# zgspose/PAVENet

Hardware: AMD Instinct MI355X
Metric: clips/sec (T=7, 800x1344) fwd (higher is better)
Workload: dtype f32 (exact 3-term bf16 split on the bf16 MFMA)

## Files before the change

### include/pave_hip.h

```cpp
#ifndef PAVE_HIP_H_
#define PAVE_HIP_H_

#include <stdint.h>

#ifdef __cplusplus
extern "C" {
#endif

#define PAVE_OK 0
#define PAVE_E_ARG (-1)
#define PAVE_E_LAUNCH (-2)
#define PAVE_E_STEP (-3)
#define PAVE_E_UNSUPPORTED (-4)

#define PAVE_ABI_VERSION 21
int pave_abi_version(void);
const char* pave_last_error(void);

int pave_ms_deform_attn_forward_f32(const float* value, const int64_t* spatial_shapes,
                                    const int64_t* level_start, const float* sampling_loc,
                                    const float* attn_weight, float* out, int bs, int S, int M,
                                    int D, int L, int Lq, int P, int im2col_step, void* stream);
int pave_ms_deform_attn_forward_f64(const double* value, const int64_t* spatial_shapes,
                                    const int64_t* level_start, const double* sampling_loc,
// ... 246 lines not shown
int pave_gemm_fp16_act_f32(const void* a, int a_is_f16, const void* w_plane, const float* bias,
                           const float* residual, const float* gamma, const float* beta, float eps, void* out,
                           int out_is_f16, long long M, int K, int N, int relu, void* stream);

int pave_gemm_bf16x3_ex_f32(const float* a, const float* a_bias, const void* w_planes,
                            const float* bias, const float* residual, long long residual_rows,
                            float* out, float* out2, int n_split, long long M, int K, int N,
                            int relu, int nplanes, void* stream);

int pave_ref_update_f32(const float* tmp, const float* ref, float* out, long long n, float eps,
                        void* stream);

int pave_groupnorm_nhwc_f32(const float* x, const float* gamma, const float* beta, float* y,
                            long long y_batch_stride, int N, int HW, int C, int G, float eps,
                            double* partial, int nchunks, float* ab, void* stream);

typedef struct pave_gn_level {
  const float* x;
  const float* gamma;
  const float* beta;
  float* y;
  long long y_batch_stride;
  int HW;
  int nchunks;
  float eps;
} pave_gn_level;
int pave_groupnorm_levels_nhwc_f32(const pave_gn_level* levels, int nlev, int N, int C, int G, double* partial,
                                   float* ab, void* stream);

int pave_gemm_bf16x3_cat_f32(const float* a, long long K1, const float* a2, const void* w_planes,
                             const float* bias, const float* residual, float* out, long long M, int K,
                             int N, int relu, int nplanes, void* stream);

int pave_gemm_bf16x3_grouped_f32(const float* a, long long lda, const void* w_planes, const float* bias,
                                 float* out, long long M, int K, int N, int group_n, int relu,
                                 int nplanes, void* stream);

int pave_gemm_bf16x3_ln_f32(const float* a, const void* w_planes, const float* bias,
                            const float* residual, const float* gamma, const float* beta, float eps,
                            float* out, long long M, int K, int N, int nplanes, void* stream);

int pave_conv3x3_split_f32(const float* x, const void* w_planes, const float* bias,
                           const float* residual, float* y, int N, int H, int W, int Cin, int Cout,
                           int stride, int relu, int nplanes, void* stream);

long long pave_conv3x3_splitk_workspace_bytes(int N, int H, int W, int Cin, int Cout, int stride);
int pave_conv3x3_splitk_f32(const float* x, const void* w_planes, const float* bias,
                            const float* residual, float* y, int N, int H, int W, int Cin, int Cout,
                            int stride, int relu, void* workspace, long long workspace_bytes,
                            int nplanes, void* stream);

long long pave_gemm_splitk_workspace_bytes(long long M, int K, int N);
int pave_gemm_bf16x3_splitk_f32(const float* a, const void* w_planes, const float* bias, const float* residual,
                                float* out, long long M, int K, int N, int relu, int nplanes, void* workspace,
                                long long workspace_bytes, void* stream);

int pave_set_form_policy(int policy);
int pave_get_form_policy(void);

#define PAVE_FORM_ROWS 0
#define PAVE_FORM_ROWS_SPLITK 1
#define PAVE_FORM_ROWS_TILE 2
#define PAVE_FORM_LN 3
#define PAVE_FORM_CONV3X3 4
#define PAVE_FORM_CONV1X1S 5
#define PAVE_FORM_ENCPROJ 6
// ... 56 lines not shown
```

### pavenet_amd/backbones.py

```python
import torch
import torch.nn as nn
import torch.nn.functional as F

from .bricks import BaseModule, build_norm_layer
from .registry import MMDET_MODELS


class BasicBlock(nn.Module):
    expansion = 1

    def __init__(self, inplanes, planes, stride=1, dilation=1, downsample=None, style='pytorch',
                 norm_cfg=dict(type='BN')):
        super().__init__()
        self.conv1 = nn.Conv2d(inplanes, planes, 3, stride, dilation, dilation, bias=False)
        self.bn1 = build_norm_layer(norm_cfg, planes)[1]
        self.conv2 = nn.Conv2d(planes, planes, 3, 1, 1, bias=False)
        self.bn2 = build_norm_layer(norm_cfg, planes)[1]
        self.relu = nn.ReLU(inplace=True)
        self.downsample = downsample
        self.pairs = (('conv1', 'bn1', True), ('conv2', 'bn2', False))


class Bottleneck(nn.Module):
    expansion = 4
# ... 50 lines not shown
        self.norm_eval = norm_eval
        self.style = style
        block, stage_blocks = self.arch_settings[depth]
        stage_blocks = stage_blocks[:num_stages]
        self.conv1 = nn.Conv2d(in_channels, stem_channels, 7, 2, 3, bias=False)
        self.bn1 = build_norm_layer(norm_cfg, stem_channels)[1]
        self.relu = nn.ReLU(inplace=True)
        self.maxpool = nn.MaxPool2d(kernel_size=3, stride=2, padding=1)
        self.res_layers = []
        inplanes = stem_channels
        for i, nb in enumerate(stage_blocks):
            planes = base_channels * 2**i
            layers = []
            for b in range(nb):
                stride = strides[i] if b == 0 else 1
                downsample = None
                if b == 0 and (stride != 1 or inplanes != planes * block.expansion):
                    downsample = nn.Sequential(
                        nn.Conv2d(inplanes, planes * block.expansion, 1, stride, bias=False),
                        build_norm_layer(norm_cfg, planes * block.expansion)[1])
                layers.append(block(inplanes, planes, stride, dilations[i], downsample, style,
                                    norm_cfg))
                inplanes = planes * block.expansion
            name = f'layer{i + 1}'
            self.add_module(name, nn.Sequential(*layers))
            self.res_layers.append(name)
        self.feat_dim = inplanes
        self._folded = None
        self.channels_last = True
        self.fused_tail_max_k = 256
        self.fused_ds_max_k = 128
        self.chain_stage64 = True
        self.chain_mode = 'full'
        self.deterministic_conv3x3 = False

    def init_weights(self):
        for m in self.modules():
            if isinstance(m, nn.Conv2d):
                nn.init.kaiming_normal_(m.weight, mode='fan_out', nonlinearity='relu')
            elif isinstance(m, (nn.BatchNorm2d, nn.GroupNorm)):
                nn.init.constant_(m.weight, 1)
                nn.init.constant_(m.bias, 0)
        for m in self.modules():
            if isinstance(m, Bottleneck):
                nn.init.constant_(m.bn3.weight, 0)
            elif isinstance(m, BasicBlock):
                nn.init.constant_(m.bn2.weight, 0)
        self._is_init = True

    def _params_key(self):
        from .bricks import SourceKey, module_tensors
        return SourceKey(module_tensors(self))

    def _stem_folded(self):
        from .bricks import SourceKey
        bn = self.bn1
        key = SourceKey([self.conv1.weight, bn.weight, bn.bias, bn.running_mean, bn.running_var])
        hit = self.__dict__.get('_stem_cache')
        if hit is None or hit[0] != key:
            mf = torch.channels_last if self.channels_last else torch.contiguous_format
            with torch.no_grad():
                hit = (key, tuple(t.contiguous(memory_format=mf) if t.dim() == 4 else t
                                  for t in _fold(self.conv1, self.bn1)))
            self.__dict__['_stem_cache'] = hit
        return hit[1]

# ... 17 lines not shown
                                and w.shape[1] % 32 == 0:
                            f[(name, bi, 'conv3_kn')] = w.flatten(1).t().contiguous()
                    if blk.downsample is not None:
                        w, b = _fold(blk.downsample[0], blk.downsample[1])
                        f[(name, bi, 'ds')] = (w.contiguous(memory_format=mf), b)
                        w3_kn = f.get((name, bi, 'conv3_kn'))
                        if w3_kn is not None and w.shape[1] % 32 == 0 and \
                                w3_kn.shape[0] + w.shape[1] <= self.fused_ds_max_k:
                            f[(name, bi, 'tail_ds_kn')] = (
                                torch.cat([w3_kn, w.flatten(1).t()], 0).contiguous(),
                                f[(name, bi, 'conv3')][1] + b)
        self._folded = (key, f)
        return f

    @staticmethod
    def _stem_split(x_nchw, w):
        from . import ops
        from .bricks import _split_cached, fused_mode, get_gemm_mode
        if not fused_mode() or torch.is_grad_enabled() or not x_nchw.is_cuda \
                or x_nchw.dtype != torch.float32 or tuple(w.shape) != (64, 3, 7, 7) \
                or x_nchw.shape[1] != 3 or x_nchw.shape[3] < 8 or not x_nchw.is_contiguous():
            return None
        wp = _split_cached(w, 'stem7x7', lambda planes: ops.split_stem7x7_weight(w.detach(), planes))
        if x_nchw.shape[3] % 4 or x_nchw.data_ptr() % 16:
            return ops.conv7x7s2_nchw_split(ops.repitch_rows(x_nchw), wp, valid_w=x_nchw.shape[3])
        return ops.conv7x7s2_nchw_split(x_nchw, wp)

    @staticmethod
    def _ds_bias(f, name, bi):
        key = (name, bi, 'ds_b3')
        if key not in f:
            f[key] = f[(name, bi, 'ds')][1] + f[(name, bi, 'conv3')][1]
        return f[key]

    @staticmethod
    def _as_rows(x):
        n, c, h, w = x.shape
        return x.permute(0, 2, 3, 1).reshape(-1, c), (n, h, w)

    @staticmethod
    def _as_map(rows, nhw):
        n, h, w = nhw
        return rows.view(n, h, w, rows.shape[-1]).permute(0, 3, 1, 2)

    def _stage64_chain_ok(self, name, x, f):
        from .bricks import _GEMM, fused_mode
        blocks = list(getattr(self, name))
        if blocks[0].downsample is not None and (name, 0, 'tail_ds_kn') not in f:
            return False
        if not (self.chain_stage64 and fused_mode() and not torch.is_grad_enabled()
                and x.is_contiguous(memory_format=torch.channels_last)
                and x.shape[0] * x.shape[2] * x.shape[3] >= _GEMM['min_rows']
                and all(isinstance(b, Bottleneck) for b in blocks)):
            return False
        for bi, blk in enumerate(blocks):
            c1, c2, c3 = blk.conv1, blk.conv2, blk.conv3
            if not (c1.out_channels == 64 and c1.stride == (1, 1)
                    and tuple(c2.weight.shape) == (64, 64, 3, 3) and c2.stride == (1, 1)
                    and c2.dilation == (1, 1) and c2.padding == (1, 1) and c2.groups == 1
                    and tuple(c3.weight.shape[:2]) == (256, 64)):
                return False
            if blk.downsample is not None and not (
                    bi == 0 and blk.downsample[0].stride == (1, 1)
                    and blk.downsample[0].in_channels == 64):
                return False
            if blk.downsample is None and c1.in_channels != 256:
# ... 54 lines not shown
        if c2.dilation[0] == 1 and c2.padding[0] == 1 and c2.stride[0] == c2.stride[1] \
                and not torch.is_grad_enabled():
            wsplit = split_conv_weight(w2)
        from .bricks import fused_mode, small_split_ok
        split3 = blk.downsample is None and (
            split_gemm_ok(rows, w3.flatten(1))
            or (wsplit is not None and fused_mode() and small_split_ok(rows, w3.flatten(1))))
        if split3:
            w3_kn = None
        if wsplit is not None:
            from .bricks import get_gemm_mode
            y = ops.conv3x3_split(y, wsplit, b2, stride=c2.stride[0], relu=True,
                                  fp16=get_gemm_mode() == 'fp16')
            b2 = None
        elif taps is not None and c2.dilation[0] == 1 and c2.padding[0] == 1:
            y = ops.conv3x3_nhwc(y, taps, b2, stride=c2.stride[0], relu=True)
            b2 = None
        else:
            y = F.conv2d(y, w2, None, c2.stride, c2.padding, c2.dilation)
            if w3_kn is None and not split3:
                ops.bias_act_rows_(y, b2, None, relu=True)
                b2 = None
        yrows, onhw = self._as_rows(y)
        if blk.downsample is not None:
            wd, bd = f[(name, bi, 'ds')]
            s = blk.downsample[0].stride[0]
            tail = f.get((name, bi, 'tail_ds_kn'))
            from .bricks import _GEMM, _split_weight, fused_mode, small_split_ok
            w3_split = b2 is None and (split_gemm_ok(yrows, w3.flatten(1)) or small_split_ok(yrows, w3.flatten(1)))
            if (s > 1 and tail is None and fused_mode() and not torch.is_grad_enabled()
                    and wd.shape[0] % 128 == 0 and wd.shape[1] % 64 == 0
                    and (yrows.shape[0] >= _GEMM['min_rows'] or w3_split)
                    and (w3_kn is not None or w3_split or split_gemm_ok(yrows, w3.flatten(1)))):
                idt = ops.conv1x1_strided_split(x, _split_weight(wd.flatten(1)),
                                                self._ds_bias(f, name, bi), stride=s)
                idt, _ = self._as_rows(idt)
                if w3_split or split_gemm_ok(yrows, w3.flatten(1)):
                    out = linear_rows(yrows, w3.flatten(1), None, relu=True, residual=idt,
                                      inplace_residual=True, a_bias=b2)
                else:
                    out = ops.rows_gemm_bias_res_act(yrows, w3_kn, None, idt, relu=True, out=idt,
                                                     a_bias=b2)
                return self._as_map(out, onhw)
            xs = x if s == 1 else x[:, :, ::s, ::s].contiguous(memory_format=torch.channels_last)
            xrows, _ = self._as_rows(xs)
            from .bricks import _split_cached
            if tail is not None and b2 is None and fused_mode() \
                    and not torch.is_grad_enabled() \
                    and tail[0].shape[0] % 32 == 0 and tail[0].shape[1] % 64 == 0 \
                    and yrows.shape[1] % 16 == 0:
                wcat = _split_cached(tail[0], 'tail_cat', lambda planes: ops.split_weight_bf16x3(
                    tail[0].t().contiguous(), planes))
                out = ops.gemm_bf16x3_cat(yrows, xrows, wcat, tail[1], None, relu=True)
            elif tail is not None:
                out = ops.rows_gemm_bias_res_act(yrows, tail[0], tail[1], None, relu=True,
                                                 a_bias=b2, a2=xrows)
            elif split_gemm_ok(xrows, wd.flatten(1)) and \
                    (w3_kn is not None or split_gemm_ok(yrows, w3.flatten(1))):
                idt = linear_rows(xrows, wd.flatten(1), self._ds_bias(f, name, bi))
                if split_gemm_ok(yrows, w3.flatten(1)):
                    out = linear_rows(yrows, w3.flatten(1), None, relu=True, residual=idt,
                                      inplace_residual=True, a_bias=b2)
                else:
                    out = ops.rows_gemm_bias_res_act(yrows, w3_kn, None, idt, relu=True, out=idt,
                                                     a_bias=b2)
            else:
# ... 412 lines not shown
```

### pavenet_amd/csrc/pave_gemm_dma.hip

```cpp
#include <hip/hip_runtime.h>
#include <type_traits>
#include <stdint.h>

#include "pave_hip.h"
#include "pave_internal.h"
#include "pave_enc_math.h"

namespace {

typedef __bf16 bf16x8 __attribute__((ext_vector_type(8)));
typedef float f32x16 __attribute__((ext_vector_type(16)));
typedef unsigned u32x4 __attribute__((ext_vector_type(4)));
typedef float f32x4 __attribute__((ext_vector_type(4)));

constexpr int QBM = 128;
constexpr int QNS = 3;
constexpr int QCST = 36;

struct QConv {
  int H, W, Cin, Ho, Wo, stride;
  unsigned rcp;
};
struct QOut {
  float* out2;
// ... 145 lines not shown
__device__ __forceinline__ void gemm_q_body(
    const float* __restrict__ A, const uint16_t* __restrict__ Wp, const float* __restrict__ bias,
    const float* residual, float* out, const int M, const int K, const int N, const int relu,
    const float* __restrict__ a_bias, const QConv g, const QOut os, const QLn ln,
    const float* __restrict__ A2 = nullptr, const int tile_m0 = -1, const int tile_n0 = 0,
    const QEpi* epi = nullptr) {
  constexpr int NWAVE = 4 * WN;
  constexpr int BN = WN * TN * 32;
  constexpr int BM = QBM * RM;
  constexpr bool AH = (IO & 1) != 0, OH = (IO & 2) != 0;
  static_assert(!AH || (PL == 1 && KIND == 0 && !ABIAS && RM == 1), "fp16 A rows: fp16 operand mode, plain rows");
  static_assert(!OH || (PL == 1 && !LNORM && EPI == 0 && !HT && RM == 1), "fp16 output: plain epilogue");
  constexpr int A_STAGE = AH ? BM * 32 : BM * 64;
  static_assert(RM == 1 || (RM == 2 && WN == 1 && !WIDE && !LNORM && EPI == 0), "two row tiles per wave: narrow form");
  static_assert(PL == 3 || PL == 1, "operand planes: 3 (bf16 split) or 1 (fp16)");
  constexpr int W_STAGE = PL * BN * 32;
  constexpr int STAGE = A_STAGE + W_STAGE;
  constexpr int NA = A_STAGE / 1024;
  constexpr int NWI = W_STAGE / 1024;
  constexpr int NDI = NA + NWI;
  constexpr int QMAX = (NDI + NWAVE - 1) / NWAVE;
  constexpr int QMIN = NDI / NWAVE;
  constexpr int QA = (NA + NWAVE - 1) / NWAVE;
  constexpr int NS = WIDE ? 2 : QNS;
  constexpr int EPI_OFF = 0;
  constexpr int STAT_OFF = NS * STAGE;
  constexpr int TQ = WIDE ? 2 : (HT ? 1 : TN);
  static_assert(!HT || (TN == 2 && WN == 1 && RM == 1 && !WIDE && !LNORM && EPI == 0 && PL == 3),
                "half-tail form: 64-column planes, one row tile per wave, 3 planes");
  static_assert(!WIDE || (TN == 8 && WN == 1 && !ABIAS), "wide form: 32 x 256 per wave");
  constexpr int ABOFF = STAT_OFF + (LNORM ? 2 * QBM * WN * 4 : 0);
  static_assert(NA % NWAVE == 0, "A DMA instructions divide evenly over the waves");
  static_assert(!LNORM || KIND == 0, "LayerNorm epilogue: plain row GEMM only");
  static_assert(KIND >= 0 && KIND <= 4, "row source");
  extern __shared__ __attribute__((aligned(1024))) unsigned char smem[];

  const int tid = threadIdx.x, lane = tid & 63;
  const int wave = __builtin_amdgcn_readfirstlane(tid >> 6);
  const int wm = wave / WN, wn = wave % WN;
  const int lr = lane & 31, kh = lane >> 5;
  const int ntiles = N / BN;
  const int ttot = ((M + BM - 1) / BM) * ntiles;
  const int per = ttot >> 3, rem = ttot & 7;
  const unsigned lds0 = (unsigned)(size_t)(__attribute__((address_space(3))) unsigned char*)smem;
  const int s0 = os.ks_slabs > 0 ? (int)blockIdx.y * os.ks_slabs : 0;
  const int nslabs = os.ks_slabs > 0 ? min(os.ks_slabs, K / 16 - s0) : K / 16;
  const long long w_slab = (long long)PL * N * 32;
  const unsigned char* const w_base = reinterpret_cast<const unsigned char*>(Wp);

  int m0 = 0, n0 = 0;
  unsigned a_voff[QA];
  unsigned a2_voff[QA];
  const unsigned char* a2_base = reinterpret_cast<const unsigned char*>(A2);
  int a_iy0[QA], a_ix0[QA];
  const float* a_img[QA];
  unsigned a_mask[QA];
  i32x4 a_rsrc;
  if (KIND == 1) {
    const unsigned long long ab = reinterpret_cast<unsigned long long>(A);
    a_rsrc.x = __builtin_amdgcn_readfirstlane((int)(unsigned)ab);
    a_rsrc.y = __builtin_amdgcn_readfirstlane((int)(unsigned)(ab >> 32) & 0xffff);
    a_rsrc.z = __builtin_amdgcn_readfirstlane(
        (int)((unsigned)(M / (g.Ho * g.Wo)) * (unsigned)g.H * (unsigned)g.W * (unsigned)g.Cin * 4u));
    a_rsrc.w = 0x00020000;
  }
  unsigned w_voff[QMAX - QA];
  const unsigned char* a_base = reinterpret_cast<const unsigned char*>(A);

  auto setup_tile = [&](const int t) {
    const int xcd = t & 7, idx = t >> 3;
    const int lb = xcd * per + (xcd < rem ? xcd : rem) + idx;
    m0 = (lb / ntiles) * BM;
    n0 = (lb % ntiles) * BN;
    if (tile_m0 >= 0) m0 = tile_m0, n0 = tile_n0;
#pragma unroll
    for (int q = 0; q < QA; ++q) {
      const int d = wave + NWAVE * q;
      const int r = AH ? d * 32 + (lane >> 1) : d * 16 + (lane >> 2);
      const int c = AH ? (lane & 1) ^ ((r >> 3) & 1) : (lane & 3) ^ ((r >> 2) & 3);
      long long gm = (long long)m0 + r;
      if (gm >= M) gm = M - 1;
      if (KIND == 0 && AH) {
        a_voff[q] = (unsigned)(((gm - m0) * (g.H > 0 ? g.H : K) + c * 8) * 2);
      } else if (KIND == 0) {
        a_voff[q] = (unsigned)(((gm - m0) * (g.H > 0 ? g.H : K) + c * 4) * 4);
      } else if (KIND == 4) {
        a_voff[q] = (unsigned)(((gm - m0) * g.Cin + c * 4) * 4);
        a2_voff[q] = (unsigned)(((gm - m0) * (K - g.Cin) + c * 4) * 4);
      } else {
        const unsigned ur = (unsigned)gm, gy = ur / (unsigned)g.Wo;
        const int ox = (int)(ur - gy * (unsigned)g.Wo);
        const int n = (int)(gy / (unsigned)g.Ho);
        const int oy = (int)(gy - (unsigned)n * (unsigned)g.Ho);
        if (KIND == 3) {
          a_voff[q] = (unsigned)(((((long long)n * g.H + oy * g.stride) * g.W + ox * g.stride) * K + c * 4) * 4);
        } else if (KIND == 1) {
          const int iy0 = oy * g.stride - 1, ix0 = ox * g.stride - 1;
          a_voff[q] = (unsigned)(((((long long)n * g.H + iy0) * g.W + ix0) * g.Cin + c * 4) * 4);
          unsigned mk = 0;
#pragma unroll
          for (int t = 0; t < 9; ++t) {
            const int iy = iy0 + t / 3, ix = ix0 + t % 3;
            mk |= (iy >= 0 && iy < g.H && ix >= 0 && ix < g.W) ? (1u << t) : 0u;
          }
          a_mask[q] = mk;
        } else {
          a_iy0[q] = oy * g.stride - 1;
          a_ix0[q] = ox * g.stride - 1;
          a_img[q] = A + (long long)n * g.H * g.W * g.Cin + c * 4;
        }
      }
    }
    if (KIND == 0 && AH)
      a_base = reinterpret_cast<const unsigned char*>(A) +
               ((long long)m0 * (g.H > 0 ? g.H : K) + (g.W > 0 ? (long long)(n0 / g.W) * K : 0)) * 2;
    else if (KIND == 0)
      a_base = reinterpret_cast<const unsigned char*>(A + (long long)(PAVE_PROBE_CACHED_A() ? 0 : m0) * (g.H > 0 ? g.H : K) +
                                                      (g.W > 0 ? (long long)(n0 / g.W) * K : 0));
    if (KIND == 4) {
      a_base = reinterpret_cast<const unsigned char*>(A + (long long)m0 * g.Cin);
      a2_base = reinterpret_cast<const unsigned char*>(A2 + (long long)m0 * (K - g.Cin));
    }
#pragma unroll
    for (int q = QA; q < QMAX; ++q) {
      const int j = wave + NWAVE * (q - QA);
      const int p = j / (NWI / PL), row = (j % (NWI / PL)) * 32 + (lane >> 1);
      const int h = (lane & 1) ^ ((row >> 3) & 1);
      w_voff[q - QA] = (unsigned)((((long long)p * N + n0 + row) * 32 + h * 16));
    }
  };
  auto issue = [&](const int rel, const int stage) {
    const int slab = rel + s0;
    const unsigned sl = lds0 + stage * STAGE;
#pragma unroll
    for (int q = 0; q < QA; ++q) {
      const unsigned dst = sl + (wave + NWAVE * q) * 1024;
      if (KIND == 1) {
        const int tap = g.rcp ? (int)__umulhi((unsigned)slab, g.rcp) : slab;
        const int c0 = (slab - tap * (g.Cin >> 4)) * 16;
        const int ky = (tap * 11) >> 5, kx = tap - ky * 3;
        const unsigned toff = (unsigned)(((ky * g.W + kx) * g.Cin + c0) * 4);
        const bool ok = (a_mask[q] >> tap) & 1u;
        dma16_buf(ok ? a_voff[q] + toff : 0xffffff00u, a_rsrc, dst);
      } else if (KIND == 2) {
        const int k0 = slab * 16;
        const int tap = k0 / g.Cin, c0 = k0 - tap * g.Cin;
        const int ky = tap / 3, kx = tap - ky * 3;
        const int iy = a_iy0[q] + ky, ix = a_ix0[q] + kx;
        const bool ok = tap < 9 && iy >= 0 && iy < g.H && ix >= 0 && ix < g.W;
        const float* src = ok ? a_img[q] + ((long long)iy * g.W + ix) * g.Cin + c0
                              : reinterpret_cast<const float*>(g_zero_chunk);
        dma16_flat(src, dst);
      } else if (KIND == 4) {
        const int s1 = g.Cin >> 4;
        if (slab < s1) dma16(a_voff[q], a_base + (long long)slab * 64, dst);
        else dma16(a2_voff[q], a2_base + (long long)(slab - s1) * 64, dst);
      } else {
        dma16(a_voff[q], a_base + (long long)slab * (AH ? 32 : 64), dst);
      }
    }
#pragma unroll
    for (int q = QA; q < QMAX; ++q) {
      const int j = wave + NWAVE * (q - QA);
      if (NWI % NWAVE == 0 || j < NWI)
        dma16(w_voff[q - QA], w_base + slab * w_slab, sl + A_STAGE + j * 1024);
    }
  };

  const int sw = (lr >> 2) & 3;
  const int a_rd0 = AH ? (wm * 32 + lr) * 32 + ((kh ^ ((lr >> 3) & 1)) * 16)
                       : (wm * 32 * RM + lr) * 64 + (((2 * kh) ^ sw) * 16);
  const int a_rd1 = a_rd0 ^ 16;
  const int w_rd = A_STAGE + (wn * TN * 32 + lr) * 32 + ((kh ^ ((lr >> 3) & 1)) * 16);

  f32x16 acc[RM * TN];
  f32x4 raw[RM][2];
  u32x4 apl[2][RM][PL];
  u32x4 wf[2][PL][TQ];
  const float* const ab_lds = reinterpret_cast<const float*>(smem + ABOFF);

  auto read_raw = [&](const int stage) {
    const unsigned char* st = smem + stage * STAGE;
#pragma unroll
    for (int rt = 0; rt < RM; ++rt) {
      raw[rt][0] = *reinterpret_cast<const f32x4*>(st + a_rd0 + rt * 2048);
      if constexpr (!AH) raw[rt][1] = *reinterpret_cast<const f32x4*>(st + a_rd1 + rt * 2048);
// ... 1310 lines not shown
      break;
    case PAVE_FORM_LN: {
      bool lnpass, sk, wide;
      ln_form(M, Kp, Np, policy, dv, &lnpass, &sk, &wide);
      if (lnpass) *order = sk ? PAVE_ORDER_KSPLIT_LNPASS : PAVE_ORDER_TILE_LNPASS;
      else *order = wide ? PAVE_ORDER_TILE : PAVE_ORDER_TILE_LN8;
      break;
    }
    case PAVE_FORM_CONV3X3:
      if (dv != PAVE_DV_FIRST_GEN) splitk_plan(M, Kp, Np, policy, &parts, &per);
      if (parts > 1) *order = PAVE_ORDER_SPLITK, *ksplit = parts;
      break;
    default:
      break;
  }
  return PAVE_OK;
}
int pave_internal_splitk_reduce(const float* ws, int parts, long long M, int n, const float* bias,
                                const float* residual, int relu, float* out, void* stream) {
  const long long total4 = M * n / 4;
  return pave_launch<splitk_reduce_kernel>(dim3((unsigned)((total4 + 255) / 256)), dim3(256), 0,
                                           reinterpret_cast<hipStream_t>(stream), ws, parts, total4, n / 4, bias,
                                           residual, relu, out);
}

template <int PL>
static int gemm_q_dispatch(const GemmQ& q) {
  const float *a = q.a, *a_bias = q.a_bias, *bias = q.bias, *residual = q.residual, *a2 = q.a2;
  float *out = q.out, *out2 = q.out2;
  const long long M = q.M;
  const int K = q.K, N = q.N, relu = q.relu, n_split = q.n_split, ks_slabs = q.ks_slabs;
  const int kind = q.rows, Ho = q.Ho, Wo = q.Wo, stride = q.stride;
  const int H = kind == GEMMQ_ROWS ? q.lda : q.H, W = kind == GEMMQ_ROWS ? q.group_n : q.W;
  const int Cin = kind == GEMMQ_ROWS2 ? q.k1 : q.Cin;
  int n_real = q.n_real, ksplit = q.ksplit;
  const QConv g{H, W, Cin, Ho, Wo, stride,
                (kind == 1 && Cin > 16) ? (unsigned)(((1ull << 32) + (Cin >> 4) - 1) / (unsigned)(Cin >> 4)) : 0u};
  if (relu < 0 || relu > 3)
    return pave_internal_fail(PAVE_E_ARG, "gemm_q: activation 0 (none), 1 (ReLU), 2 (GELU) or 3 (sigmoid)");
  const bool narrow = q.narrow_groups;
  if (n_real <= 0) n_real = N;
  if (n_real > N || n_real % 4 != 0 || (out2 && n_real != N))
    return pave_internal_fail(PAVE_E_ARG, "gemm_q: n_real %% 4 == 0, n_real <= N (== N with two outputs)");
  if (ksplit > 1 && (bias || residual || out2 || a_bias || relu || ks_slabs < 4 || ks_slabs % 2 != 0 ||
                     (long long)(ksplit - 1) * ks_slabs + 4 > K / 16 || (long long)ksplit * ks_slabs < K / 16))
    return pave_internal_fail(PAVE_E_ARG, "gemm_q: split-K parts are raw partial sums of >= 4 slabs");
  if (ksplit < 1) ksplit = 1;
  const QOut os{out2, out2 ? n_split : 0, q.residual_rows >= M ? 0 : (int)q.residual_rows, n_real,
                ksplit > 1 ? ks_slabs : 0};
  hipStream_t st = reinterpret_cast<hipStream_t>(q.stream);
  const uint16_t* w = static_cast<const uint16_t*>(q.w_planes);
  if (K % 32 != 0 || K < 64) return pave_internal_fail(PAVE_E_ARG, "gemm_q: K %% 32 == 0, K >= 64");
  if ((os.res_rows != 0 && (long long)os.res_rows * n_real * 4 >= (1ll << 31)) || (long long)N * 512 >= (1ll << 31))
    return pave_internal_fail(PAVE_E_ARG, "gemm_q: row-periodic table of >= 2 GiB, or rows of >= 16 MiB");
  if (kind != 1 && K >= (1 << 23))
    return pave_internal_fail(PAVE_E_ARG, "gemm_q: K < 2^23 (32-bit lane offsets inside a 128-row tile)");
  if (a_bias && (kind != 0 || K > 8192))
    return pave_internal_fail(PAVE_E_ARG, "gemm_q: a_bias with the plain row form, K <= 8192");
  if (kind == 1 && Cin % 16 != 0) return pave_internal_fail(PAVE_E_ARG, "gemm_q: 3x3 form needs Cin %% 16 == 0");
  if (kind == 4 && (!a2 || Cin <= 0 || Cin >= K || Cin % 16 != 0))
    return pave_internal_fail(PAVE_E_ARG, "gemm_q: two-source rows need a2 and 0 < K1 < K, K1 %% 16 == 0");
  const int dv = pave_internal_diag_variant();
  if (kind == 0 && rows_ksplit(M, N, K, pave_internal_form_policy()) && !a_bias && !out2 && ksplit == 1 &&
      (dv == PAVE_DV_NONE || dv == PAVE_DV_SK_ANY_ROWS)) {
    if (M > kSkRows && dv != PAVE_DV_SK_ANY_ROWS && (W <= 0 || W % (32 * kSkmTiles) == 0))
      return launch_skm<PL>(a, w, bias, residual, out, M, K, N, relu, H > 0 ? H : K, W > 0 ? W : 0, os.res_rows,
                            n_real, st);
    return launch_sk<PL>(a, w, bias, residual, out, M, K, N, relu, H > 0 ? H : K, W > 0 ? W : 0, os.res_rows,
                         n_real, st);
  }
  if (kind == 0 && small_rows_form(M, N) && N <= 512 && !a_bias && !out2 && ksplit == 1 &&
      (dv == PAVE_DV_NONE || dv == PAVE_DV_SMALL_ROWS_R5))
    return launch_s<1, 4, PL>(a, w, bias, residual, out, M, K, N, relu, H > 0 ? H : K, W > 0 ? W : 0, os.res_rows,
                          n_real, st);
  const bool big3 = kind == 1 && ((M / ((long long)Ho * Wo)) * H * W * Cin * 4 >= (1ll << 32) - 65536 ||
                                  dv == PAVE_DV_CONV3_ADDR64);
#define PAVE_QGO(TN_)                                                                               \
  if (kind == 0) {                                                                                  \
    if (a_bias) return launch_q<TN_, 0, true, 1, PL>(a, w, bias, residual, out, M, K, N, relu, a_bias, st, g, os); \
    return launch_q<TN_, 0, false, 1, PL>(a, w, bias, residual, out, M, K, N, relu, a_bias, st, g, os, nullptr, ksplit); \
  }                                                                                                 \
  if (kind == 1 && big3) return launch_q<TN_, 2, false, 1, PL>(a, w, bias, residual, out, M, K, N, relu, a_bias, st, g, os, nullptr, ksplit); \
  if (kind == 1) return launch_q<TN_, 1, false, 1, PL>(a, w, bias, residual, out, M, K, N, relu, a_bias, st, g, os, nullptr, ksplit); \
  if (kind == 4) return launch_q<TN_, 4, false, 1, PL>(a, w, bias, residual, out, M, K, N, relu, a_bias, st, g, os, a2, ksplit); \
  return launch_q<TN_, 3, false, 1, PL>(a, w, bias, residual, out, M, K, N, relu, a_bias, st, g, os, nullptr, ksplit)
  const long long wtiles = ((M + QBM - 1) / QBM) * (N / 256) * ksplit;
  if (N % 256 == 0 && n_real == N && !narrow && !a_bias && dv != PAVE_DV_WIDE_NEVER &&
      (wtiles >= 400 || dv == PAVE_DV_WIDE_ALWAYS) &&
      !(kind == 0 && W > 0 && W % 256 != 0) && (!out2 || n_split % 256 == 0)) {
    if (kind == 0) return launch_w<0, PL>(a, w, bias, residual, out, M, K, N, relu, st, g, os, nullptr, ksplit);
    if (kind == 1 && big3) return launch_w<2, PL>(a, w, bias, residual, out, M, K, N, relu, st, g, os, nullptr, ksplit);
    if (kind == 1) return launch_w<1, PL>(a, w, bias, residual, out, M, K, N, relu, st, g, os, nullptr, ksplit);
    if (kind == 4) return launch_w<4, PL>(a, w, bias, residual, out, M, K, N, relu, st, g, os, a2, ksplit);
    return launch_w<3, PL>(a, w, bias, residual, out, M, K, N, relu, st, g, os, nullptr, ksplit);
// ... 264 lines not shown
```

### pavenet_amd/csrc/pave_gemm_split.hip

```cpp
#include <hip/hip_runtime.h>
#include <stdint.h>

#include "pave_hip.h"
#include "pave_internal.h"

namespace {

typedef __bf16 bf16x8 __attribute__((ext_vector_type(8)));
typedef float f32x16 __attribute__((ext_vector_type(16)));
typedef unsigned u32x4 __attribute__((ext_vector_type(4)));
typedef float f32x4 __attribute__((ext_vector_type(4)));
typedef float f32x4_u __attribute__((ext_vector_type(4), aligned(4)));

constexpr int BK = 16;
constexpr int RST = 48;

__device__ __forceinline__ int stage_row_perm(int r) {
  return (r & ~7) | ((r & 3) << 1) | ((r >> 2) & 1);
}

__device__ __forceinline__ unsigned hi16(float x) { return __float_as_uint(x) & 0xffff0000u; }
__device__ __forceinline__ unsigned pack_hi(unsigned lo, unsigned hi) {
  return __builtin_amdgcn_perm(hi, lo, 0x07060302u);
}
// ... 583 lines not shown
  return parts > 1 ? (long long)parts * M * N * 4 : 0;
}

int pave_gemm_bf16x3_splitk_f32(const float* a, const void* w_planes, const float* bias, const float* residual,
                                float* out, long long M, int K, int N, int relu, int nplanes, void* workspace,
                                long long workspace_bytes, void* stream) {
  if (!a || !w_planes || !out || !workspace || (relu != 0 && relu != 1))
    return pave_internal_fail(PAVE_E_ARG, "gemm_bf16x3_splitk: null pointer (or relu not 0 | 1)");
  if (!q_planes(nplanes)) return pave_internal_fail(PAVE_E_ARG, "gemm_bf16x3_splitk: nplanes must be 3 or PAVE_PLANES_FP16");
  const long long need = pave_gemm_splitk_workspace_bytes(M, K, N);
  if (need == 0 || workspace_bytes < need)
    return pave_internal_fail(PAVE_E_ARG, "gemm_bf16x3_splitk: shape has no split-K plan (use pave_gemm_bf16x3_f32) or "
                                          "the workspace is smaller than pave_gemm_splitk_workspace_bytes");
  int parts, per;
  pave_internal_splitk_plan(M, K, (N + 63) / 64 * 64, &parts, &per);
  float* ws = static_cast<float*>(workspace);
  GemmQ q = gemm_q_call(a, w_planes, nullptr, nullptr, ws, M, K, N, 0, nplanes, stream);
  q.ksplit = parts, q.ks_slabs = per;
  const int rc = pave_internal_gemm_q(q);
  if (rc != PAVE_OK) return rc;
  return pave_internal_splitk_reduce(ws, parts, M, N, bias, residual, relu, out, stream);
}

int pave_gemm_fp16_act_f32(const void* a, int a_is_f16, const void* w_plane, const float* bias,
                           const float* residual, const float* gamma, const float* beta, float eps, void* out,
                           int out_is_f16, long long M, int K, int N, int relu, void* stream) {
  if (!a || !w_plane || !out) return pave_internal_fail(PAVE_E_ARG, "gemm_fp16_act: null pointer");
  if (M <= 0 || M >= (1ll << 31) || K <= 0 || N <= 0)
    return pave_internal_fail(PAVE_E_ARG, "gemm_fp16_act: bad sizes (0 < M < 2^31)");
  return pave_internal_gemm_f16act(a, a_is_f16 != 0, w_plane, bias, residual, gamma, beta, eps, out, out_is_f16 != 0,
                                   M, K, N, relu, stream);
}

int pave_gemm_bf16x3_cat_f32(const float* a, long long K1, const float* a2, const void* w_planes,
                             const float* bias, const float* residual, float* out, long long M, int K,
                             int N, int relu, int nplanes, void* stream) {
  if (!a || !a2 || !w_planes || !out) return pave_internal_fail(PAVE_E_ARG, "gemm_bf16x3_cat: null pointer");
  if (M <= 0 || M >= (1ll << 31) || K <= 0 || N <= 0)
    return pave_internal_fail(PAVE_E_ARG, "gemm_bf16x3_cat: bad sizes (0 < M < 2^31)");
  if (K % 32 != 0 || K < 64 || N % 64 != 0 || K1 <= 0 || K1 >= K || K1 % 16 != 0)
    return pave_internal_fail(PAVE_E_ARG, "gemm_bf16x3_cat: K %% 32 == 0, N %% 64 == 0, 0 < K1 < K, K1 %% 16 == 0");
  if (!q_planes(nplanes)) return pave_internal_fail(PAVE_E_ARG, "gemm_bf16x3_cat: nplanes must be 3 or PAVE_PLANES_FP16");
  GemmQ q = gemm_q_call(a, w_planes, bias, residual, out, M, K, N, relu, nplanes, stream);
  q.rows = GEMMQ_ROWS2, q.a2 = a2, q.k1 = (int)K1;
  return pave_internal_gemm_q(q);
}

int pave_gemm_bf16x3_grouped_f32(const float* a, long long lda, const void* w_planes, const float* bias,
                                 float* out, long long M, int K, int N, int group_n, int relu,
                                 int nplanes, void* stream) {
  if (!a || !w_planes || !out) return pave_internal_fail(PAVE_E_ARG, "gemm_bf16x3_grouped: null pointer");
  if (M <= 0 || M >= (1ll << 31) || K <= 0 || N <= 0 || group_n <= 0)
    return pave_internal_fail(PAVE_E_ARG, "gemm_bf16x3_grouped: bad sizes (0 < M < 2^31)");
  if (K % 32 != 0 || K < 64 || N % group_n != 0 || group_n % 64 != 0 ||
      lda < (long long)(N / group_n) * K || lda % 4 != 0 || lda >= (1ll << 23))
    return pave_internal_fail(PAVE_E_ARG, "gemm_bf16x3_grouped: K %% 32 == 0, group_n %% 64 == 0, N %% group_n == 0, "
                                          "groups * K <= lda < 2^23 (a tile's 127 rows x lda x 4 B is a 32-bit lane offset), lda %% 4 == 0");
  if (!q_planes(nplanes)) return pave_internal_fail(PAVE_E_ARG, "gemm_bf16x3_grouped: nplanes must be 3 or PAVE_PLANES_FP16");
  GemmQ q = gemm_q_call(a, w_planes, bias, nullptr, out, M, K, N, relu, nplanes, stream);
  q.lda = (int)lda, q.group_n = group_n;
  q.narrow_groups = !(N % 128 == 0 && group_n % 128 == 0);
  return pave_internal_gemm_q(q);
}

int pave_gemm_bf16x3_ln_f32(const float* a, const void* w_planes, const float* bias,
                            const float* residual, const float* gamma, const float* beta, float eps,
                            float* out, long long M, int K, int N, int nplanes, void* stream) {
  if (!a || !w_planes || !out || !gamma || !beta)
    return pave_internal_fail(PAVE_E_ARG, "gemm_bf16x3_ln: null pointer");
  if (M <= 0 || K <= 0 || M >= (1ll << 31))
    return pave_internal_fail(PAVE_E_ARG, "gemm_bf16x3_ln: bad sizes (0 < M < 2^31)");
  if (K % 64 != 0 || N != 256)
    return pave_internal_fail(PAVE_E_UNSUPPORTED, "gemm_bf16x3_ln: K %% 64 == 0 and N == 256 required");
  if (!q_planes(nplanes)) return pave_internal_fail(PAVE_E_ARG, "gemm_bf16x3_ln: nplanes must be 3 or PAVE_PLANES_FP16");
  if (g_diag_variant != PAVE_DV_FIRST_GEN || nplanes != 3)
    return pave_internal_gemm_q_ln(a, w_planes, bias, residual, gamma, beta, eps, out, M, K, N, stream,
                                   q_planes(nplanes));
  return launch_gemm<2, 2, false, 3, false, false, true, 4, true>(
// ... 149 lines not shown
```

### pavenet_amd/csrc/pave_internal.h

```cpp
#ifndef PAVE_INTERNAL_H_
#define PAVE_INTERNAL_H_
#include <type_traits>

int pave_internal_fail(int code, const char* msg);

template <auto KERN, class... A>
inline int pave_launch(dim3 grid, dim3 block, int smem, hipStream_t st, A... args) {
  hipLaunchKernelGGL(KERN, grid, block, smem, st, args...);
  const hipError_t e = hipGetLastError();
  if (e != hipSuccess) return pave_internal_fail(PAVE_E_LAUNCH, hipGetErrorString(e));
  return PAVE_OK;
}
template <auto KERN, class... A>
inline int pave_launch_lds(const char* refusal, dim3 grid, dim3 block, int smem, hipStream_t st, A... args) {
  static int raised = 0;
  if (smem > raised) {
    if (hipFuncSetAttribute(reinterpret_cast<const void*>(KERN), hipFuncAttributeMaxDynamicSharedMemorySize,
                            smem) != hipSuccess)
      return pave_internal_fail(PAVE_E_LAUNCH, refusal);
    raised = smem;
  }
  return pave_launch<KERN>(grid, block, smem, st, args...);
}

// ... 6 lines not shown
  PAVE_DV_NO_SPLITK = 6,
  PAVE_DV_WIDE_ALWAYS = 7,
  PAVE_DV_WIDE_NEVER = 8,
  PAVE_DV_FIRST_GEN = 9,
  PAVE_DV_LN_8WAVE = 13,
  PAVE_DV_LN_WIDE = 14,
  PAVE_DV_RM2_NEVER = 15,
  PAVE_DV_RM2_ALWAYS = 16,
  PAVE_DV_NO_HALF_TAIL = 17,
  PAVE_DV_SWIN_PER_LANE = 18,
  PAVE_DV_SMALL_ROWS_R5 = 19,
  PAVE_DV_WIDE_ONE_PER_CU = 20,
  PAVE_DV_SK_ANY_ROWS = 21,
};
#ifdef PAVE_DIAG
int pave_internal_diag_variant();
#else
static inline int pave_internal_diag_variant() { return PAVE_DV_NONE; }
#endif

static inline int q_planes(int nplanes) { return nplanes == 3 ? 3 : (nplanes == PAVE_PLANES_FP16 ? 1 : 0); }
template <class F>
inline int pave_with_planes(int planes, const char* refusal, F f) {
  if (planes == 1) return f(std::integral_constant<int, 1>{});
  if (planes != 3) return pave_internal_fail(PAVE_E_ARG, refusal);
  return f(std::integral_constant<int, 3>{});
}

enum GemmQRows : int {
  GEMMQ_ROWS = 0,
  GEMMQ_CONV3X3 = 1,
  GEMMQ_CONV1X1S = 3,
  GEMMQ_ROWS2 = 4,
};
struct GemmQ {
  GemmQRows rows = GEMMQ_ROWS;
  const float* a = nullptr;
  const float* a2 = nullptr;
  const float* a_bias = nullptr;
  const void* w_planes = nullptr;
  const float* bias = nullptr;
  const float* residual = nullptr;
  long long residual_rows = 0;
  float* out = nullptr;
  float* out2 = nullptr;
  int n_split = 0;
  long long M = 0;
  int K = 0, N = 0;
  int n_real = 0;
  int relu = 0;
  int lda = 0, group_n = 0;
  bool narrow_groups = false;
  int H = 0, W = 0, Cin = 0, Ho = 0, Wo = 0, stride = 0;
  int k1 = 0;
  int ksplit = 1, ks_slabs = 0;
  int planes = 3;
  void* stream = nullptr;
};
int pave_internal_gemm_q(const GemmQ& q);
void pave_internal_splitk_plan(long long M, int Kp, int Np, int* ksplit, int* ks_slabs);
int pave_internal_form_policy();
int pave_internal_splitk_reduce(const float* ws, int parts, long long M, int n, const float* bias,
                                const float* residual, int relu, float* out, void* stream);
int pave_internal_gemm_q_ln(const float* a, const void* w_planes, const float* bias, const float* residual,
                            const float* gamma, const float* beta, float eps, float* out, long long M,
                            int K, int N, void* stream, int planes = 3);
// ... 10 lines not shown
```

### pavenet_amd/ops.py

```python
import contextlib
import ctypes

import torch

from . import native


KERNEL_EVENTS = None
KERNEL_EVENT_TAGS = ('enc_tile', 'enc_grid_T1')
KERNEL_EVENT_SHAPES = None


def _stream_ptr():
    return torch.cuda.current_stream().cuda_stream


FORM_ROWS, FORM_ROWS_SPLITK, FORM_ROWS_TILE, FORM_LN, FORM_CONV3X3, FORM_CONV1X1S, FORM_ENCPROJ = (
    native.DEFINES['PAVE_FORM_' + n] for n in ('ROWS', 'ROWS_SPLITK', 'ROWS_TILE', 'LN', 'CONV3X3', 'CONV1X1S',
                                               'ENCPROJ'))
ORDER_TILE, ORDER_KSPLIT, ORDER_SPLITK, ORDER_TILE_LNPASS, ORDER_KSPLIT_LNPASS, ORDER_TILE_LN8 = (
    native.DEFINES['PAVE_ORDER_' + n] for n in ('TILE', 'KSPLIT', 'SPLITK', 'TILE_LNPASS', 'KSPLIT_LNPASS',
                                                'TILE_LN8'))


# ... 1123 lines not shown
    if out is None:
        out = torch.empty((M, N), dtype=torch.float32, device=a.device)
    else:
        _dev(out, 'out', torch.float32)
        _require(tuple(out.shape) == (M, N), 'gemm_bf16x3: out [M,N]')
    if N % 256 == 0 and npl in _Q_PLANES and a_bias is None and N == w_planes.shape[2]:
        M1 = round_split_rows(M, N // 256)
        if M1 is not None:
            gemm_bf16x3(a[:M1], w_planes, bias, residual[:M1] if residual is not None else None, relu=relu,
                        out=out[:M1], fp16=fp16)
            gemm_bf16x3(a[M1:], w_planes, bias, residual[M1:] if residual is not None else None, relu=relu,
                        out=out[M1:], fp16=fp16)
            return out
    ws_bytes = lib.pave_gemm_splitk_workspace_bytes(M, K, N) \
        if (SPLITK_ROWS and K >= 2048 and M < 200 * 128 and npl in _Q_PLANES and a_bias is None
            and relu in (False, True, 0, 1)) else 0
    if ws_bytes > 0:
        ws = torch.empty(ws_bytes // 4, dtype=torch.float32, device=a.device)
        _launch('pave_gemm_bf16x3_splitk_f32', 'gemm_bf16x3_splitk', a.device,
                a.data_ptr(), w_planes.data_ptr(), _ptr(bias), _ptr(residual),
                out.data_ptr(), M, K, N, int(bool(relu)), npl, ws.data_ptr(), ws_bytes,
                tag=_gemm_tag('gemm_bf16x3', M), flops=2 * M * K * N,
                shape=(M, K, N, 'relu' if relu else '', 'res' if residual is not None else '', 'split-K'))
        return out
    _launch('pave_gemm_bf16x3_f32', 'gemm_bf16x3', a.device,
            a.data_ptr(), _ptr(a_bias), w_planes.data_ptr(), _ptr(bias),
            _ptr(residual), out.data_ptr(), M, K, N, _ACT_CODE.get(relu, int(bool(relu))), npl,
            tag=_gemm_tag('gemm_bf16x3', M), flops=2 * M * K * N,
            shape=(M, K, N, 'relu' if relu else '', 'res' if residual is not None else '',
                   'abias' if a_bias is not None else ''))
    return out


def gemm_bf16x3_cat(a, a2, w_planes, bias=None, residual=None, relu=False, out=None):
    _dev(a, 'a', torch.float32)
    _dev(a2, 'a2', torch.float32)
    npl = _planes(w_planes, only=_Q_PLANES)
    _require(a.dim() == 2 and a2.dim() == 2 and a.shape[0] == a2.shape[0],
             'gemm_bf16x3_cat: a [M, K1], a2 [M, K2]')
    M, K1 = a.shape
    K = K1 + a2.shape[1]
    _require(w_planes.shape[0] * 16 == K, 'gemm_bf16x3_cat: w_planes [(K1+K2)/16, 3, N, 16]')
    N = w_planes.shape[2]
    _require(K % 32 == 0 and N % 64 == 0 and K1 % 16 == 0, 'gemm_bf16x3_cat: K % 32, N % 64, K1 % 16')
    if bias is not None:
        _dev(bias, 'bias', torch.float32)
        _require(bias.numel() == N, 'gemm_bf16x3_cat: bias [N]')
    if residual is not None:
        _dev(residual, 'residual', torch.float32)
        _require(tuple(residual.shape) == (M, N), 'gemm_bf16x3_cat: residual [M, N]')
    if out is None:
        out = torch.empty((M, N), dtype=torch.float32, device=a.device)
    else:
        _dev(out, 'out', torch.float32)
        _require(tuple(out.shape) == (M, N), 'gemm_bf16x3_cat: out [M, N]')
    _launch('pave_gemm_bf16x3_cat_f32', 'gemm_bf16x3_cat', a.device,
            a.data_ptr(), K1, a2.data_ptr(), w_planes.data_ptr(), _ptr(bias), _ptr(residual), out.data_ptr(), M, K, N,
            int(bool(relu)), npl,
            tag=_gemm_tag('gemm_bf16x3', M), flops=2 * M * K * N, shape=(M, K, N, 'cat', f'k1={K1}'))
    return out


def gemm_bf16x3_grouped(a, w_planes, bias, group_n, relu=False):
    _dev(a, 'a', torch.float32)
    npl = _planes(w_planes, only=_Q_PLANES)
    _require(a.dim() == 2, 'gemm_bf16x3_grouped: a [M, G*K], w_planes [K/16, 3, N, 16]')
    M, lda = a.shape
    K, N = w_planes.shape[0] * 16, w_planes.shape[2]
    G = N // int(group_n)
    _require(G * group_n == N and G * K == lda, 'gemm_bf16x3_grouped: a has G*K columns, N = G*group_n')
    if bias is not None:
        _dev(bias, 'bias', torch.float32)
        _require(bias.numel() == N, 'gemm_bf16x3_grouped: bias [N]')
    out = torch.empty((M, N), dtype=torch.float32, device=a.device)
    _launch('pave_gemm_bf16x3_grouped_f32', 'gemm_bf16x3_grouped', a.device,
            a.data_ptr(), lda, w_planes.data_ptr(), _ptr(bias), out.data_ptr(), M, K, N, int(group_n),
            int(bool(relu)), npl,
            tag=_gemm_tag('gemm_bf16x3', M), flops=2 * M * K * N, shape=(M, K, N, 'grouped', f'g{G}'))
    return out


def conv1x1_strided_split(x, w_planes, bias=None, stride=2, relu=False):
    _nhwc(x, 'conv1x1_strided_split')
    npl = _planes(w_planes, only=_Q_PLANES)
    N, Cin, H, W = x.shape
    _require(w_planes.shape[0] * 16 == Cin, 'conv1x1_strided_split: w_planes [Cin/16, 3, Cout, 16]')
    Cout = w_planes.shape[2]
    if bias is not None:
# ... 502 lines not shown
```

Measured before the change: 59.42.

## Fuse strided downsample 1x1 into bottleneck conv3 GEMM at stage boundaries

At a stride-2 stage boundary, the conv3 1x1 GEMM and the strided downsample 1x1 conv now run as one concatenated-K GEMM. A new row-source kind lets the DMA A-loader read rows from the conv3 input and strided pixels directly from the NHWC block input. This removes a separate kernel launch and the write and read-back of the identity tensor. It adds a new kernel variant restricted to the wide form (N % 256), plus cached concatenated weight splits.

```diff
diff --git a/include/pave_hip.h b/include/pave_hip.h
--- a/include/pave_hip.h
+++ b/include/pave_hip.h
@@ -302,6 +302,10 @@
                              const float* bias, const float* residual, float* out, long long M, int K,
                              int N, int relu, int nplanes, void* stream);
 
+int pave_gemm_bf16x3_cat_strided_f32(const float* a, long long K1, const float* a2, int N, int H, int W, int C2,
+                                     int stride, const void* w_planes, const float* bias, float* out, int Cout,
+                                     int relu, int nplanes, void* stream);
+
 int pave_gemm_bf16x3_grouped_f32(const float* a, long long lda, const void* w_planes, const float* bias,
                                  float* out, long long M, int K, int N, int group_n, int relu,
                                  int nplanes, void* stream);
diff --git a/pavenet_amd/backbones.py b/pavenet_amd/backbones.py
--- a/pavenet_amd/backbones.py
+++ b/pavenet_amd/backbones.py
@@ -106,6 +106,7 @@
         self.fused_ds_max_k = 128
         self.chain_stage64 = True
         self.chain_mode = 'full'
+        self.fuse_stage_boundary = True
         self.deterministic_conv3x3 = False
 
     def init_weights(self):
@@ -189,6 +190,23 @@
         if key not in f:
             f[key] = f[(name, bi, 'ds')][1] + f[(name, bi, 'conv3')][1]
         return f[key]
+
+    @staticmethod
+    def _boundary_operands(f, name, bi):
+        key = (name, bi, 'tail_ds_nk')
+        if key not in f:
+            f[key] = (torch.cat([f[(name, bi, 'conv3')][0].flatten(1), f[(name, bi, 'ds')][0].flatten(1)], 1)
+                      .contiguous(), ResNet._ds_bias(f, name, bi))
+        return f[key]
+
+    def _boundary_fused_ok(self, yrows, x, w3, wd, s):
+        from . import ops
+        k1, c2 = w3.shape[1], wd.shape[1]
+        return (s == 2 and yrows.shape[0] >= ops.SMALL_ROWS and self.fuse_stage_boundary
+                and wd.shape[0] % 256 == 0 and k1 % 16 == 0 and c2 % 16 == 0 and (k1 + c2) % 64 == 0
+                and x.numel() * 4 < 2 ** 32 and x.dtype == torch.float32
+                and x.is_contiguous(memory_format=torch.channels_last)
+                and ops.current_form_policy() == 0)
 
     @staticmethod
     def _as_rows(x):
@@ -309,6 +327,13 @@
                     and wd.shape[0] % 128 == 0 and wd.shape[1] % 64 == 0
                     and (yrows.shape[0] >= _GEMM['min_rows'] or w3_split)
                     and (w3_kn is not None or w3_split or split_gemm_ok(yrows, w3.flatten(1)))):
+                if b2 is None and w3_split and self._boundary_fused_ok(yrows, x, w3, wd, s):
+                    wcat, bcat = self._boundary_operands(f, name, bi)
+                    from .bricks import _split_cached
+                    out = ops.gemm_bf16x3_cat(yrows, x, _split_cached(
+                        wcat, 'tail_cat_s', lambda planes: ops.split_weight_bf16x3(wcat, planes)),
+                        bcat, None, relu=True, stride=s)
+                    return self._as_map(out, onhw)
                 idt = ops.conv1x1_strided_split(x, _split_weight(wd.flatten(1)),
                                                 self._ds_bias(f, name, bi), stride=s)
                 idt, _ = self._as_rows(idt)
diff --git a/pavenet_amd/csrc/pave_gemm_dma.hip b/pavenet_amd/csrc/pave_gemm_dma.hip
--- a/pavenet_amd/csrc/pave_gemm_dma.hip
+++ b/pavenet_amd/csrc/pave_gemm_dma.hip
@@ -201,7 +201,8 @@
   constexpr int ABOFF = STAT_OFF + (LNORM ? 2 * QBM * WN * 4 : 0);
   static_assert(NA % NWAVE == 0, "A DMA instructions divide evenly over the waves");
   static_assert(!LNORM || KIND == 0, "LayerNorm epilogue: plain row GEMM only");
-  static_assert(KIND >= 0 && KIND <= 4, "row source");
+  static_assert(KIND >= 0 && KIND <= 5, "row source");
+  static_assert(KIND != 5 || WIDE, "rows + strided pixels: wide form only");
   extern __shared__ __attribute__((aligned(1024))) unsigned char smem[];
 
   const int tid = threadIdx.x, lane = tid & 63;
@@ -256,6 +257,14 @@
       } else if (KIND == 4) {
         a_voff[q] = (unsigned)(((gm - m0) * g.Cin + c * 4) * 4);
         a2_voff[q] = (unsigned)(((gm - m0) * (K - g.Cin) + c * 4) * 4);
+      } else if (KIND == 5) {
+        const unsigned ur = (unsigned)gm, gy = ur / (unsigned)g.Wo;
+        const int ox = (int)(ur - gy * (unsigned)g.Wo);
+        const int n = (int)(gy / (unsigned)g.Ho);
+        const int oy = (int)(gy - (unsigned)n * (unsigned)g.Ho);
+        a_voff[q] = (unsigned)(((gm - m0) * g.Cin + c * 4) * 4);
+        a2_voff[q] =
+            (unsigned)(((((long long)n * g.H + oy * g.stride) * g.W + ox * g.stride) * (K - g.Cin) + c * 4) * 4);
       } else {
         const unsigned ur = (unsigned)gm, gy = ur / (unsigned)g.Wo;
         const int ox = (int)(ur - gy * (unsigned)g.Wo);
@@ -290,6 +299,7 @@
       a_base = reinterpret_cast<const unsigned char*>(A + (long long)m0 * g.Cin);
       a2_base = reinterpret_cast<const unsigned char*>(A2 + (long long)m0 * (K - g.Cin));
     }
+    if (KIND == 5) a_base = reinterpret_cast<const unsigned char*>(A + (long long)m0 * g.Cin);
 #pragma unroll
     for (int q = QA; q < QMAX; ++q) {
       const int j = wave + NWAVE * (q - QA);
@@ -320,7 +330,7 @@
         const float* src = ok ? a_img[q] + ((long long)iy * g.W + ix) * g.Cin + c0
                               : reinterpret_cast<const float*>(g_zero_chunk);
         dma16_flat(src, dst);
-      } else if (KIND == 4) {
+      } else if (KIND == 4 || KIND == 5) {
         const int s1 = g.Cin >> 4;
         if (slab < s1) dma16(a_voff[q], a_base + (long long)slab * 64, dst);
         else dma16(a2_voff[q], a2_base + (long long)(slab - s1) * 64, dst);
@@ -1697,7 +1707,7 @@
   const int K = q.K, N = q.N, relu = q.relu, n_split = q.n_split, ks_slabs = q.ks_slabs;
   const int kind = q.rows, Ho = q.Ho, Wo = q.Wo, stride = q.stride;
   const int H = kind == GEMMQ_ROWS ? q.lda : q.H, W = kind == GEMMQ_ROWS ? q.group_n : q.W;
-  const int Cin = kind == GEMMQ_ROWS2 ? q.k1 : q.Cin;
+  const int Cin = (kind == GEMMQ_ROWS2 || kind == GEMMQ_ROWS2S) ? q.k1 : q.Cin;
   int n_real = q.n_real, ksplit = q.ksplit;
   const QConv g{H, W, Cin, Ho, Wo, stride,
                 (kind == 1 && Cin > 16) ? (unsigned)(((1ull << 32) + (Cin >> 4) - 1) / (unsigned)(Cin >> 4)) : 0u};
@@ -1725,6 +1735,18 @@
   if (kind == 1 && Cin % 16 != 0) return pave_internal_fail(PAVE_E_ARG, "gemm_q: 3x3 form needs Cin %% 16 == 0");
   if (kind == 4 && (!a2 || Cin <= 0 || Cin >= K || Cin % 16 != 0))
     return pave_internal_fail(PAVE_E_ARG, "gemm_q: two-source rows need a2 and 0 < K1 < K, K1 %% 16 == 0");
+  if (kind == GEMMQ_ROWS2S) {
+    if (!a2 || Cin <= 0 || Cin >= K || Cin % 16 != 0 || (K - Cin) % 16 != 0 || H <= 0 || W <= 0 ||
+        (stride != 1 && stride != 2) || Ho != (H - 1) / stride + 1 || Wo != (W - 1) / stride + 1 ||
+        M % ((long long)Ho * Wo) != 0 || residual || a_bias || out2 || ksplit != 1 || q.residual_rows != 0)
+      return pave_internal_fail(PAVE_E_ARG, "gemm_q: rows + strided pixels need a2, 0 < K1 < K, K1 and K - K1 %% 16 "
+                                            "== 0, stride 1 or 2, M = images x Ho x Wo, no residual / second output");
+    if (N % 256 != 0 || n_real != N)
+      return pave_internal_fail(PAVE_E_UNSUPPORTED, "gemm_q: rows + strided pixels need N %% 256 == 0 (wide form)");
+    if ((M / ((long long)Ho * Wo)) * H * W * (K - Cin) * 4 >= (1ll << 32))
+      return pave_internal_fail(PAVE_E_UNSUPPORTED, "gemm_q: rows + strided pixels need a map below 4 GiB");
+    return launch_w<5, PL>(a, w, bias, nullptr, out, M, K, N, relu, st, g, os, a2, 1);
+  }
   const int dv = pave_internal_diag_variant();
   if (kind == 0 && rows_ksplit(M, N, K, pave_internal_form_policy()) && !a_bias && !out2 && ksplit == 1 &&
       (dv == PAVE_DV_NONE || dv == PAVE_DV_SK_ANY_ROWS)) {
diff --git a/pavenet_amd/csrc/pave_gemm_split.hip b/pavenet_amd/csrc/pave_gemm_split.hip
--- a/pavenet_amd/csrc/pave_gemm_split.hip
+++ b/pavenet_amd/csrc/pave_gemm_split.hip
@@ -639,6 +639,18 @@
                                    M, K, N, relu, stream);
 }
 
+static int gemm_cat_entry(const float* a, long long K1, const float* a2, int H, int W, int stride,
+                          const void* w_planes, const float* bias, const float* residual, float* out, long long M,
+                          int K, int N, int relu, int nplanes, void* stream) {
+  GemmQ q = gemm_q_call(a, w_planes, bias, residual, out, M, K, N, relu, nplanes, stream);
+  q.rows = GEMMQ_ROWS2, q.a2 = a2, q.k1 = (int)K1;
+  if (H > 0) {
+    q.rows = GEMMQ_ROWS2S, q.H = H, q.W = W, q.stride = stride;
+    q.Ho = (H - 1) / stride + 1, q.Wo = (W - 1) / stride + 1;
+  }
+  return pave_internal_gemm_q(q);
+}
+
 int pave_gemm_bf16x3_cat_f32(const float* a, long long K1, const float* a2, const void* w_planes,
                              const float* bias, const float* residual, float* out, long long M, int K,
                              int N, int relu, int nplanes, void* stream) {
@@ -648,9 +660,27 @@
   if (K % 32 != 0 || K < 64 || N % 64 != 0 || K1 <= 0 || K1 >= K || K1 % 16 != 0)
     return pave_internal_fail(PAVE_E_ARG, "gemm_bf16x3_cat: K %% 32 == 0, N %% 64 == 0, 0 < K1 < K, K1 %% 16 == 0");
   if (!q_planes(nplanes)) return pave_internal_fail(PAVE_E_ARG, "gemm_bf16x3_cat: nplanes must be 3 or PAVE_PLANES_FP16");
-  GemmQ q = gemm_q_call(a, w_planes, bias, residual, out, M, K, N, relu, nplanes, stream);
-  q.rows = GEMMQ_ROWS2, q.a2 = a2, q.k1 = (int)K1;
-  return pave_internal_gemm_q(q);
+  return gemm_cat_entry(a, K1, a2, 0, 0, 0, w_planes, bias, residual, out, M, K, N, relu, nplanes, stream);
+}
+
+int pave_gemm_bf16x3_cat_strided_f32(const float* a, long long K1, const float* a2, int N, int H, int W, int C2,
+                                     int stride, const void* w_planes, const float* bias, float* out, int Cout,
+                                     int relu, int nplanes, void* stream) {
+  if (!a || !a2 || !w_planes || !out) return pave_internal_fail(PAVE_E_ARG, "gemm_bf16x3_cat_strided: null pointer");
+  if (N <= 0 || H <= 0 || W <= 0 || (stride != 1 && stride != 2) || (relu != 0 && relu != 1))
+    return pave_internal_fail(PAVE_E_ARG, "gemm_bf16x3_cat_strided: bad sizes (stride 1 or 2; relu 0 | 1)");
+  if (K1 <= 0 || K1 >= (1 << 22) || K1 % 16 != 0 || C2 <= 0 || C2 >= (1 << 22) || C2 % 16 != 0 ||
+      (K1 + C2) % 32 != 0 || K1 + C2 < 64 || Cout <= 0)
+    return pave_internal_fail(PAVE_E_ARG, "gemm_bf16x3_cat_strided: K1 %% 16 == 0, C2 %% 16 == 0, (K1 + C2) %% 32 == 0, "
+                                          "K1 + C2 >= 64");
+  if (!q_planes(nplanes))
+    return pave_internal_fail(PAVE_E_ARG, "gemm_bf16x3_cat_strided: nplanes must be 3 or PAVE_PLANES_FP16");
+  const long long M = (long long)N * ((H - 1) / stride + 1) * ((W - 1) / stride + 1);
+  if (M >= (1ll << 31)) return pave_internal_fail(PAVE_E_ARG, "gemm_bf16x3_cat_strided: tensor too large");
+  if ((long long)N * H * W * C2 * 4 >= (1ll << 32))
+    return pave_internal_fail(PAVE_E_UNSUPPORTED, "gemm_bf16x3_cat_strided: the a2 map must be smaller than 4 GiB");
+  return gemm_cat_entry(a, K1, a2, H, W, stride, w_planes, bias, nullptr, out, M, (int)(K1 + C2), Cout, relu, nplanes,
+                        stream);
 }
 
 int pave_gemm_bf16x3_grouped_f32(const float* a, long long lda, const void* w_planes, const float* bias,
diff --git a/pavenet_amd/csrc/pave_internal.h b/pavenet_amd/csrc/pave_internal.h
--- a/pavenet_amd/csrc/pave_internal.h
+++ b/pavenet_amd/csrc/pave_internal.h
@@ -62,6 +62,7 @@
   GEMMQ_CONV3X3 = 1,
   GEMMQ_CONV1X1S = 3,
   GEMMQ_ROWS2 = 4,
+  GEMMQ_ROWS2S = 5,
 };
 struct GemmQ {
   GemmQRows rows = GEMMQ_ROWS;
diff --git a/pavenet_amd/ops.py b/pavenet_amd/ops.py
--- a/pavenet_amd/ops.py
+++ b/pavenet_amd/ops.py
@@ -1179,14 +1179,22 @@
     return out
 
 
-def gemm_bf16x3_cat(a, a2, w_planes, bias=None, residual=None, relu=False, out=None):
+def gemm_bf16x3_cat(a, a2, w_planes, bias=None, residual=None, relu=False, out=None, stride=None):
     _dev(a, 'a', torch.float32)
-    _dev(a2, 'a2', torch.float32)
     npl = _planes(w_planes, only=_Q_PLANES)
-    _require(a.dim() == 2 and a2.dim() == 2 and a.shape[0] == a2.shape[0],
-             'gemm_bf16x3_cat: a [M, K1], a2 [M, K2]')
+    _require(a.dim() == 2, 'gemm_bf16x3_cat: a [M, K1]')
     M, K1 = a.shape
-    K = K1 + a2.shape[1]
+    if stride is None:
+        _dev(a2, 'a2', torch.float32)
+        _require(a2.dim() == 2 and a2.shape[0] == M, 'gemm_bf16x3_cat: a [M, K1], a2 [M, K2]')
+        K2 = a2.shape[1]
+    else:
+        _nhwc(a2, 'gemm_bf16x3_cat')
+        B, K2, H, W = a2.shape
+        _require(stride in (1, 2) and residual is None, 'gemm_bf16x3_cat: a2 map at stride 1 or 2, no residual')
+        _require(M == B * ((H - 1) // stride + 1) * ((W - 1) // stride + 1),
+                 'gemm_bf16x3_cat: a has one row per strided pixel of a2')
+    K = K1 + K2
     _require(w_planes.shape[0] * 16 == K, 'gemm_bf16x3_cat: w_planes [(K1+K2)/16, 3, N, 16]')
     N = w_planes.shape[2]
     _require(K % 32 == 0 and N % 64 == 0 and K1 % 16 == 0, 'gemm_bf16x3_cat: K % 32, N % 64, K1 % 16')
@@ -1201,6 +1209,12 @@
     else:
         _dev(out, 'out', torch.float32)
         _require(tuple(out.shape) == (M, N), 'gemm_bf16x3_cat: out [M, N]')
+    if stride is not None:
+        _launch('pave_gemm_bf16x3_cat_strided_f32', 'gemm_bf16x3_cat_strided', a.device,
+                a.data_ptr(), K1, a2.data_ptr(), B, H, W, K2, int(stride), w_planes.data_ptr(), _ptr(bias),
+                out.data_ptr(), N, int(bool(relu)), npl,
+                tag=_gemm_tag('gemm_bf16x3', M), flops=2 * M * K * N, shape=(M, K, N, 'relu' if relu else '', '', ''))
+        return out
     _launch('pave_gemm_bf16x3_cat_f32', 'gemm_bf16x3_cat', a.device,
             a.data_ptr(), K1, a2.data_ptr(), w_planes.data_ptr(), _ptr(bias), _ptr(residual), out.data_ptr(), M, K, N,
             int(bool(relu)), npl,
```

After: 59.73 (median of 6 runs). About the same (+0.5%).
